# OpenDriveLab/OccNet

Hardware: AMD Instinct MI355X
Metric: nuScenes samples/sec (6-cam 900x1600 -> 200x200x16 voxels) (higher is better)
Workload: dtype f32 hot path (GEMM operands bf16x3-split, SCA value rows q16 block floating point) + bf16 backbone; 1 GPU; bevformer_base_occ forward: 6x(3x928x1600) images -> ResNet-50+FPN -> 4 BEVFormer layers (TSA+SCA+FFN) -> lifter + 2xConv3d decoder -> 200x200x16 voxels x (17 logits + 2 flow); history_frames=0, mode=infer, scope=e2e, input=resident-f32, samples_per_gpu=1, global_batch=1, parallelism=dp1, step_graph=False, linear_precision=bf16x3, backbone_dtype=bf16

## Files before the change

include/occnet_amd.h:

```cpp
#ifndef OCCNET_AMD_H_
#define OCCNET_AMD_H_

#include <stdint.h>

#ifdef __cplusplus
extern "C" {
#endif

#define OCC_OK 0
#define OCC_E_INVALID (-1)
#define OCC_E_LAUNCH (-2)
#define OCC_E_UNSUPPORTED (-3)

int occ_abi_version(void);
const char* occ_last_error(void);
int occ_selftest_fdiv_f32(const float* a, const float* d, float* q, int64_t n, void* stream);


int occ_ms_deform_attn_forward_f32(const float* value, const int64_t* spatial_shapes,
                                   const int64_t* level_start_index, const float* sampling_loc,
                                   const float* attn_weight, float* out, int B, int S, int M, int D,
                                   int L, int Lq, int P, int im2col_step, void* stream);

int occ_ms_deform_attn_backward_f32(const float* value, const int64_t* spatial_shapes,
// ... 200 lines not shown
                                    float* scale_out, void* stream);

int occ_value_proj_bf16_planes(int n_segments, const void* const* a, const int64_t* lda, const int64_t* rows,
                               const int64_t* rows_per_group, const int64_t* out_row0,
                               const float* const* group_bias, int bias_groups, const void* weight_packed, void* out,
                               int out_f16, int64_t ldo, int K, int n_planes, int plane_cols, int64_t plane_stride,
                               int64_t out_group_rows, const float* out_scale, void* stream);

int occ_stem_conv7x7_pool_f32_bf16(const float* x, const void* weight_frag, const float* bias, void* out,
                                   int batch, int H, int W, void* stream);
int occ_stem_conv7x7_pool_u8_bf16(const uint8_t* x, const void* weight_frag, const float* bias, void* out,
                                  int batch, int Hs, int Ws, int H, int W, const float* mean,
                                  const float* std, int to_rgb, void* stream);

int occ_bias_relu_maxpool_nhwc_bf16(const void* y, const float* bias, void* out, int batch, int H, int W, int C,
                                    void* stream);

int occ_conv1x1_nhwc_bf16(const void* x, const void* weight, const float* bias, const void* residual,
                          void* out, int batch, int Hin, int Win, int Cin, int Cout, int stride, int relu,
                          int residual_upsample2, void* stream);

int occ_conv1x1_nhwc_bf16_variant(const void* x, const void* weight, const float* bias, const void* residual,
                                  void* out, int batch, int Hin, int Win, int Cin, int Cout, int stride, int relu,
                                  int residual_upsample2, int variant, void* stream);

int64_t occ_conv1x1_wgrad_workspace_bytes(int N, int H, int W, int Cin, int Cout, int stride, int splits);
int occ_conv1x1_wgrad_nhwc_bf16(const void* g, const void* x, void* dw, int dw_bf16, void* workspace, int N, int H, int W,
                                int Cin, int Cout, int stride, int splits, void* stream);

int64_t occ_conv3x3_wgrad_workspace_bytes(int N, int H, int W, int Cin, int Cout, int stride, int splits);
int occ_conv3x3_wgrad_nhwc_bf16(const void* g, const void* x, void* dw, int dw_bf16, void* workspace, int N, int H, int W,
                                int Cin, int Cout, int stride, int splits, void* stream);

int occ_conv3x3_pack_weight_bf16(const float* weight, void* packed, int Cout, int Cin, void* stream);
int occ_conv3x3_nhwc_bf16(const void* x, const void* weight_packed, const float* bias, void* out, int batch,
                          int H, int W, int Cin, int Cout, int stride, int relu, void* stream);
int occ_conv3x3_nhwc_bf16_amax(const void* x, const void* weight_packed, const float* bias, void* out, int batch,
                               int H, int W, int Cin, int Cout, int stride, int relu, uint32_t* amax8, void* stream);
int occ_conv3x3_nhwc_bf16_variant(const void* x, const void* weight_packed, const float* bias, void* out, int batch,
                                  int H, int W, int Cin, int Cout, int stride, int relu, uint32_t* amax8, int variant,
                                  void* stream);

int occ_conv3x3_conv1x1_nhwc_bf16(const void* x, const void* w3x3_packed, const float* b2, const void* w1x1_frag,
                                  const float* b3, const void* residual, void* out, int batch, int H, int W, int Cmid,
                                  int Cout, int stride, int variant, void* stream);
int occ_conv3x3_conv1x1_pick(int batch, int H, int W, int Cmid, int Cout, int stride);

int occ_mfma_pack_b_frag_bf16(const float* weight, void* packed, int N, int K, void* stream);

int occ_bottleneck64_nhwc_bf16(const void* x, const void* w1_frag, const float* b1, const void* w2_frag,
                               const float* b2, const void* w3_frag, const float* b3, void* out, int batch,
                               int H, int W, int Cin, int downsample, void* stream);

int64_t occ_ray_metrics_state_words(int free_id);
int64_t occ_ray_metrics_workspace_bytes(int B, int X, int Y, int Z);
int occ_ray_metrics_accumulate(const void* sem_pred, int sem_pred_dtype, const float* flow_pred,
                               const void* sem_gt, int sem_gt_dtype, const float* flow_gt,
                               const float* origins, const int32_t* origin_counts, const float* rays,
                               float off_x, float off_y, float off_z, float voxel_size, int free_id,
                               int64_t* state, float* rows_pred, float* rows_gt, void* workspace,
                               int64_t workspace_bytes, int B, int Tmax, int X, int Y, int Z, int R,
                               void* stream);

int64_t occ_heads_loss_workspace_bytes(int64_t n_rows, int num_classes, int max_blocks);
int occ_heads_loss_fwd_f32(const float* feat, const float* w1_occ, const float* b1_occ, const float* w2_occ,
                           const float* b2_occ, const float* w1_flow, const float* b1_flow, const float* w2_flow,
                           const float* b2_flow, const void* labels, int labels_dtype, const float* flow_gt,
                           const uint8_t* mask, const float* class_weight, int64_t ignore_index, int reduction_mean,
                           float* losses, void* workspace, int64_t workspace_bytes, int64_t n_rows, int C, int hidden,
                           int num_classes, int max_blocks, void* stream);
int occ_heads_loss_bwd_f32(const float* feat, const float* w1_occ, const float* b1_occ, const float* w2_occ,
                           const float* b2_occ, const float* w1_flow, const float* b1_flow, const float* w2_flow,
                           const float* b2_flow, const void* labels, int labels_dtype, const float* flow_gt,
                           const uint8_t* mask, const float* class_weight, int64_t ignore_index, int reduction_mean,
                           const float* grad_losses, const float* occ_denom, float* dfeat, float* dw1_occ,
                           float* db1_occ, float* dw2_occ, float* db2_occ, float* dw1_flow, float* db1_flow,
                           float* dw2_flow, float* db2_flow, void* workspace, int64_t workspace_bytes, int64_t n_rows,
                           int C, int hidden, int num_classes, int max_blocks, void* stream);

#ifdef __cplusplus
}
#endif
#endif
```

occnet_amd/csrc/bottleneck64_nhwc_bf16.hip:

```cpp
#include "common.h"

namespace occ {

constexpr int kBnTH = 8, kBnTW = 16, kBnHH = 10, kBnHW = 18, kBnNP = kBnHH * kBnHW;
constexpr int kBnXS = 80;
constexpr int kBnXA = 192 * kBnXS;
constexpr int kBnMS = 144;
constexpr int kBnH1ROW = kBnHW * kBnMS;
constexpr int kBnH1 = kBnHH * kBnH1ROW;
constexpr int kBnC2 = 128 * kBnMS;
constexpr int kBnOLD = 256 + 4;

__global__ void mfma_pack_b_frag_kernel(const float* __restrict__ w, unsigned short* __restrict__ packed,
                                        int N, int K) {
  const long n_el = (long)N * K;
  const long idx = (long)blockIdx.x * blockDim.x + threadIdx.x;
  if (idx >= n_el) return;
  const int j = (int)(idx & 7), lane = (int)((idx >> 3) & 63);
  const long rest = idx >> 9;
  const int nts = N / 32;
  const int nt = (int)(rest % nts), ks = (int)(rest / nts);
  const int n = nt * 32 + (lane & 31), k = ks * 16 + (lane >> 5) * 8 + j;
  packed[idx] = bf16_rne(w[(long)n * K + k]);
}
// ... 215 lines not shown
      DST[rr] = *reinterpret_cast<const uint2*>(xs + (((long)img * H + cy) * W + cx) * CIN + c);  \
    }                                                                                             \
  }
  OCC_BN_ISSUE_RES(rn, 0)
#pragma unroll
  for (int rt = 0; rt < 4; ++rt) {
    __syncthreads();
#pragma unroll
    for (int t = 0; t < 2; ++t)
#pragma unroll
      for (int r = 0; r < 16; ++r)
        sO[((r & 3) + 8 * (r >> 2) + 4 * kb) * kBnOLD + (wave * 2 + t) * 32 + vi] = acc3[rt][t][r];
#pragma unroll
    for (int rr = 0; rr < 8; ++rr) rv[rr] = rn[rr];
    if (rt + 1 < 4) OCC_BN_ISSUE_RES(rn, rt + 1)
    __syncthreads();
#pragma unroll
    for (int rr = 0; rr < 8; ++rr) {
      const int row = wave * 8 + rr;
      const int oy = y0 + 2 * rt + (row >> 4), ox = x0 + (row & 15);
      if (oy < H && ox < W) {
        float4 v = *reinterpret_cast<const float4*>(sO + row * kBnOLD + c);
        v.x += bv.x + bf16_to_f32((unsigned short)(rv[rr].x & 0xffffu));
        v.y += bv.y + bf16_to_f32((unsigned short)(rv[rr].x >> 16));
        v.z += bv.z + bf16_to_f32((unsigned short)(rv[rr].y & 0xffffu));
        v.w += bv.w + bf16_to_f32((unsigned short)(rv[rr].y >> 16));
        v.x = fmaxf(v.x, 0.f); v.y = fmaxf(v.y, 0.f); v.z = fmaxf(v.z, 0.f); v.w = fmaxf(v.w, 0.f);
        const uint2 o = make_uint2(pack_bf16x2_rne(v.x, v.y), pack_bf16x2_rne(v.z, v.w));
        *reinterpret_cast<uint2*>(out + (((long)img * H + oy) * W + ox) * 256 + c) = o;
      }
    }
  }
#undef OCC_BN_ISSUE_RES
}

}

extern "C" int occ_mfma_pack_b_frag_bf16(const float* weight, void* packed, int N, int K, void* stream) {
  using namespace occ;
  OCC_CHECK_ARG(weight && packed, "mfma_pack_b_frag_bf16: null pointer argument");
  OCC_CHECK_ARG(N > 0 && K > 0, "mfma_pack_b_frag_bf16: bad dimension");
  if (N % 32 || K % 16) {
    set_error("mfma_pack_b_frag_bf16: N=%d K=%d (need N %% 32 == 0, K %% 16 == 0)", N, K);
    return OCC_E_UNSUPPORTED;
  }
  const long n = (long)N * K;
  hipLaunchKernelGGL(mfma_pack_b_frag_kernel, dim3((unsigned)((n + 255) / 256)), dim3(256), 0,
                     reinterpret_cast<hipStream_t>(stream), weight, reinterpret_cast<unsigned short*>(packed),
                     N, K);
  OCC_CHECK_LAUNCH("mfma_pack_b_frag_bf16");
  return OCC_OK;
}

extern "C" int occ_bottleneck64_nhwc_bf16(const void* x, const void* w1_frag, const float* b1,
                                          const void* w2_frag, const float* b2, const void* w3_frag,
                                          const float* b3, void* out, int batch, int H, int W, int Cin,
                                          int downsample, void* stream) {
  using namespace occ;
  OCC_CHECK_ARG(x && w1_frag && b1 && w2_frag && b2 && w3_frag && b3 && out,
                "bottleneck64_nhwc_bf16: null pointer argument");
  OCC_CHECK_ARG(batch > 0 && H > 0 && W > 0, "bottleneck64_nhwc_bf16: bad dimension");
  if (!((Cin == 256 && !downsample) || (Cin == 64 && downsample))) {
    set_error("bottleneck64_nhwc_bf16: no kernel for Cin=%d downsample=%d (256/identity or 64/projection)", Cin,
              downsample);
    return OCC_E_UNSUPPORTED;
  }
  const int tiles_x = (W + kBnTW - 1) / kBnTW, tiles_y = (H + kBnTH - 1) / kBnTH;
  hipStream_t st = reinterpret_cast<hipStream_t>(stream);
  const unsigned gx = (unsigned)((long)batch * tiles_x * tiles_y);
#define OCC_BN_LAUNCH(CINN, DSS)                                                                     \
  hipLaunchKernelGGL((bottleneck64_nhwc_bf16_kernel<CINN, DSS>), dim3(gx), dim3(256), 0, st,            \
                     reinterpret_cast<const uint4*>(x), reinterpret_cast<const uint4*>(w1_frag), b1,    \
                     reinterpret_cast<const uint4*>(w2_frag), b2, reinterpret_cast<const uint4*>(w3_frag), \
                     b3, reinterpret_cast<unsigned short*>(out), H, W, tiles_x, tiles_y)
  if (downsample) OCC_BN_LAUNCH(64, true); else OCC_BN_LAUNCH(256, false);
#undef OCC_BN_LAUNCH
  OCC_CHECK_LAUNCH("bottleneck64_nhwc_bf16");
  return OCC_OK;
}
```

occnet_amd/ext.py:

```python
import ctypes
import os

import torch

from . import _lib, cache_epoch
from ._lib import OccAmdError, OccAmdUnsupported, f32, i32, i64, ptr, stream_ptr


_TIMING = None
_TIMING_ONLY = None


def kernel_timing(enable=True):
    global _TIMING, _TIMING_ONLY
    _TIMING = {} if enable else None
    _TIMING_ONLY = None
    return _TIMING


def kernel_timing_only(names):
    global _TIMING_ONLY
    _TIMING_ONLY = None if names is None else set(names)


# ... 1895 lines not shown
        rc = lib.occ_conv1x1_wgrad_nhwc_bf16(ptr(g), ptr(x), ptr(dw), i32(1 if out_dtype == torch.bfloat16 else 0), ptr(ws),
                                             i32(N), i32(H), i32(W), i32(Cin), i32(Cout), i32(s), i32(sp),
                                             stream_ptr(x.device))
    _note_flops('bb_conv1x1_wgrad', 2.0 * N * g.shape[2] * g.shape[3] * Cin * Cout)
    _lib.check(rc, "conv1x1_wgrad_nhwc")
    return dw


def conv1x1_dgrad_nhwc(g, w16):
    _need_cl_bf16("conv1x1_dgrad_nhwc", "g", g)
    if not (isinstance(w16, torch.Tensor) and w16.is_cuda and w16.is_floating_point() and w16.dim() in (2, 4)
            and w16.shape[0] == g.shape[1] and w16.numel() == w16.shape[0] * w16.shape[1] and w16.device == g.device):
        raise OccAmdUnsupported("conv1x1_dgrad_nhwc: w16 must be a (Cout, Cin, 1, 1) device weight matching g's channels")
    O, I = w16.shape[0], w16.shape[1]
    with torch.cuda.device(g.device), _timed('bb_conv1x1_dgrad'):
        frag = conv1x1_pack_weight(w16.reshape(O, I).t())
        gx = conv1x1_nhwc(g, frag, torch.zeros(I, dtype=torch.float32, device=g.device), _timing=None)
    _note_flops('bb_conv1x1_dgrad', 2.0 * g.shape[0] * g.shape[2] * g.shape[3] * I * O)
    return gx


def mfma_pack_b_frag(weight2d):
    _need_cuda_f32("weight", weight2d)
    if weight2d.dim() != 2:
        raise OccAmdError("mfma_pack_b_frag: expected a (N, K) matrix")
    weight2d = weight2d.contiguous()
    n, k = weight2d.shape
    packed = torch.empty(n * k, dtype=torch.int16, device=weight2d.device)
    with torch.cuda.device(weight2d.device):
        rc = _lib.lib().occ_mfma_pack_b_frag_bf16(ptr(weight2d), ptr(packed), i32(n), i32(k),
                                                  stream_ptr(weight2d.device))
    _lib.check(rc, "mfma_pack_b_frag")
    return packed


def bottleneck64_pack(w1, b1, w2, b2, w3, b3, wds=None, bds=None):
    w1 = w1.float().reshape(w1.shape[0], -1)
    w3 = w3.float().reshape(w3.shape[0], -1)
    if tuple(w2.shape) != (64, 64, 3, 3) or w1.shape[0] != 64 or tuple(w3.shape) != (256, 64):
        raise OccAmdUnsupported("bottleneck64_pack: only 64 mid / 256 output channels")
    ds = wds is not None
    cin = w1.shape[1]
    if (ds and cin != 64) or (not ds and cin != 256):
        raise OccAmdUnsupported("bottleneck64_pack: Cin must be 256 (identity) or 64 (projection)")
    w2m = w2.float().permute(0, 2, 3, 1).reshape(64, 9 * 64)
    b3 = b3.float()
    if ds:
        w3 = torch.cat([w3, wds.float().reshape(256, 64)], dim=1)
        b3 = b3 + bds.float()
    return dict(w1=mfma_pack_b_frag(w1), b1=b1.float().contiguous(), w2=mfma_pack_b_frag(w2m),
                b2=b2.float().contiguous(), w3=mfma_pack_b_frag(w3), b3=b3.contiguous(), cin=cin, ds=ds)


def bottleneck64_nhwc(x, pack):
    _need_cl_bf16("bottleneck64_nhwc", "x", x)
    N, Cin, H, W = x.shape
    if Cin != pack['cin']:
        raise OccAmdError("bottleneck64_nhwc: x has %d channels, the pack was built for %d" % (Cin, pack['cin']))
    out = torch.empty((N, 256, H, W), dtype=torch.bfloat16, device=x.device, memory_format=torch.channels_last)
    with torch.cuda.device(x.device), _timed('bb_bottleneck64'):
        rc = _lib.lib().occ_bottleneck64_nhwc_bf16(ptr(x), ptr(pack['w1']), ptr(pack['b1']), ptr(pack['w2']),
                                                   ptr(pack['b2']), ptr(pack['w3']), ptr(pack['b3']), ptr(out),
                                                   i32(N), i32(H), i32(W), i32(Cin), i32(1 if pack['ds'] else 0),
                                                   stream_ptr(x.device))
    _note_flops('bb_bottleneck64', 2.0 * N * H * W * (Cin * 64 + 9 * 64 * 64 + 64 * 256 + (Cin * 256 if pack['ds'] else 0)))
    _lib.check(rc, "bottleneck64_nhwc")
    return out


def conv3x3_pack_weight(weight):
    _need_cuda_f32("weight", weight)
    if weight.dim() != 4 or tuple(weight.shape[2:]) != (3, 3):
        raise OccAmdError("conv3x3_pack_weight: expected a (Cout, Cin, 3, 3) weight")
    cout, cin = weight.shape[:2]
    packed = torch.empty(weight.numel(), dtype=torch.int16, device=weight.device)
    with torch.cuda.device(weight.device):
        rc = _lib.lib().occ_conv3x3_pack_weight_bf16(ptr(weight), ptr(packed), i32(cout), i32(cin),
                                                     stream_ptr(weight.device))
    _lib.check(rc, "conv3x3_pack_weight")
    return packed


def conv3x3_nhwc(x, w_packed, bias, cout, relu=False, stride=1, amax=None, variant=None):
    return _conv3x3_nhwc(x, w_packed, bias, cout, relu, stride, amax, variant, 'bb_conv3x3')


def _conv3x3_nhwc(x, w_packed, bias, cout, relu, stride, amax, variant, timing):
    _need_cl_bf16("conv3x3_nhwc", "x", x)
    _need_cuda_f32("bias", bias)
    N, Cin, H, W = x.shape
    if w_packed.numel() != cout * Cin * 9 or bias.numel() != cout:
        raise OccAmdError("conv3x3_nhwc: inconsistent shapes")
    st = int(stride)
    if st not in (1, 2):
        raise OccAmdUnsupported("conv3x3_nhwc: stride must be 1 or 2")
    if amax is not None and not (amax.is_cuda and amax.dtype == torch.int32 and amax.numel() == 8 and amax.is_contiguous()):
        raise OccAmdError("conv3x3_nhwc: amax must be 8 contiguous int32 device words")
    out = torch.empty((N, cout, (H - 1) // st + 1, (W - 1) // st + 1), dtype=torch.bfloat16, device=x.device,
                      memory_format=torch.channels_last)
    with torch.cuda.device(x.device), _timed(timing):
        rc = _lib.lib().occ_conv3x3_nhwc_bf16_variant(ptr(x), ptr(w_packed), ptr(bias), ptr(out), i32(N), i32(H),
                                                      i32(W), i32(Cin), i32(cout), i32(st), i32(1 if relu else 0),
                                                      ptr(amax), i32(0 if variant is None else int(variant)),
                                                      stream_ptr(x.device))
    _note_flops(timing, 2.0 * N * out.shape[2] * out.shape[3] * 9 * Cin * cout)
    _lib.check(rc, "conv3x3_nhwc")
    return out


def conv3x3_wgrad_nhwc(g, x, stride=1, out_dtype=torch.float32, splits=None):
    _need_cl_bf16("conv3x3_wgrad_nhwc", "g", g)
    _need_cl_bf16("conv3x3_wgrad_nhwc", "x", x)
    if out_dtype not in (torch.float32, torch.bfloat16):
        raise OccAmdUnsupported("conv3x3_wgrad_nhwc: out_dtype must be float32 or bfloat16")
    N, Cin, H, W = x.shape
    s = int(stride)
    Cout = g.shape[1]
# ... 74 lines not shown
```

occnet_amd/plugin/backbone_plan.py:

```python
import os

import torch
import torch.nn as nn
import torch.nn.functional as F
from torch.nn.utils.fusion import fuse_conv_bn_weights

from .. import ext
from .._lib import OccAmdUnsupported

_CL = torch.channels_last


def own_conv_kind(weight_shape, stride, padding, dilation=(1, 1), groups=1):
    cout, cin, kh, kw = weight_shape
    stride, padding = tuple(stride), tuple(padding)
    if tuple(dilation) != (1, 1) or groups != 1 or cin % 32:
        return None
    if (kh, kw) == (1, 1) and padding == (0, 0) and stride[0] == stride[1] and cout % 32 == 0:
        return '1x1'
    if (kh, kw) == (3, 3) and padding == (1, 1) and stride in ((1, 1), (2, 2)) and cout % 128 == 0:
        return '3x3'
    return None


# ... 112 lines not shown
            y = y + b.to(y.dtype).view(1, -1, 1, 1)
        else:
            y = F.conv2d(x, w, b.to(w.dtype), c.stride, c.padding, c.dilation, c.groups)
        if add is not None:
            y = y.add_(add)
        return y.relu_() if (relu or add is not None) else y

    @torch.no_grad()
    def forward(self, x):
        if not self.use_graph or not x.is_cuda:
            return self._forward_eager(x)
        key = (tuple(x.shape), x.dtype, str(x.device))
        st = self._graphs.setdefault(key, dict(calls=0))
        st['calls'] += 1
        if st['calls'] <= 2:
            return self._forward_eager(x)
        if 'graph' not in st:
            st['in'] = x.clone()
            torch.cuda.synchronize(x.device)
            g = torch.cuda.CUDAGraph()
            with torch.cuda.graph(g):
                st['out'] = self._forward_eager(st['in'])
            st['graph'] = g
        st['in'].copy_(x)
        st['graph'].replay()
        return st['out']

    def forward_u8(self, x_u8, mean, std, to_rgb=False, size_divisor=32):
        if not self._stem_fused:
            raise OccAmdUnsupported("forward_u8 needs the fused stem kernel (bf16 plan, 7x7/s2 stem + 3x3/s2 pool)")
        x, hw = ext.stem_conv7x7_pool_u8(x_u8, self.stem_frag, self.stem.bias, mean, std,
                                         to_rgb=to_rgb, size_divisor=size_divisor)
        return self._forward_stages(x), hw

    def _forward_eager(self, x):
        stem = self.stem
        if self._stem_fused and x.is_cuda and x.dtype == torch.float32 and x.is_contiguous():
            return self._forward_stages(ext.stem_conv7x7_pool(x, self.stem_frag, stem.bias))
        x = x.to(self.dtype).contiguous(memory_format=_CL)
        if self.hip_tail and stem.cout % 8 == 0 and x.is_cuda:
            y = F.conv2d(x, stem.weight, None, stem.stride, stem.padding, stem.dilation, stem.groups)
            if y.is_contiguous(memory_format=_CL):
                x = ext.bias_relu_maxpool_nhwc(y, stem.bias)
            else:
                x = F.max_pool2d((y + stem.bias.to(y.dtype).view(1, -1, 1, 1)).relu_(), kernel_size=3, stride=2, padding=1)
        else:
            x = F.max_pool2d(self._conv(stem, x, relu=True), kernel_size=3, stride=2, padding=1)
        return self._forward_stages(x)

    def _run_stage(self, si, x):
        for bi, (c1, c2, c3, ds) in enumerate(self.stages[si]):
            whole = self._bneck.get((si, bi))
            if whole is not None and x.is_contiguous(memory_format=_CL):
                x = ext.bottleneck64_nhwc(x, whole)
                continue
            identity = x if ds is None else self._conv(ds, x)
            y = self._conv(c1, x, relu=True)
            fused = self._conv23_fused(c2, c3, y, identity)
            x = fused if fused is not None else self._conv(c3, self._conv(c2, y, relu=True), add=identity)
        return x

    def _conv23_fused(self, c2, c3, y, identity):
        if not (c2.kind == '3x3' and c3.kind == '1x1') or os.environ.get('OCC_CONV3X3_FUSE_1X1', '1').startswith('0'):
            return None
        if not (y.is_cuda and y.dtype == torch.bfloat16 and y.is_contiguous(memory_format=_CL)
                and identity.dtype == torch.bfloat16 and identity.is_contiguous(memory_format=_CL)):
            return None
        cmid, stride = c2.cout, c2.stride[0]
        if c3.stride != (1, 1) or c3.weight.shape[1] != cmid:
            return None
        n, _, h, w = y.shape
        if not ext.conv3x3_conv1x1_pick(n, h, w, cmid, c3.cout, stride):
            return None
        return ext.conv3x3_conv1x1_nhwc(y, c2.pack, c2.bias, cmid, c3.pack, c3.bias, identity, stride=stride)

    @torch.no_grad()
    def forward_prefix(self, x):
        x = ext.stem_conv7x7_pool(x, self.stem_frag, self.stem.bias)
        for si in range(len(self.stages)):
            x = self._run_stage(si, x)
        return x

    def _forward_stages(self, x):
        feats = []
        for si in range(len(self.stages)):
            x = self._run_stage(si, x)
            if si in self.out_indices:
                feats.append(x)
        nk = self.neck
        inputs = feats
        n = len(self.laterals)
        lat = [None] * n
        nearest = nk.upsample_cfg.get('mode', 'nearest') == 'nearest' and 'scale_factor' not in nk.upsample_cfg
        for i in range(n - 1, -1, -1):
            xin = inputs[i + nk.start_level]
            li = self.laterals[i]
            up = lat[i + 1] if i + 1 < n else None
            if up is not None and nearest and li.kind == '1x1' and xin.shape[2] == 2 * up.shape[2] \
                    and xin.shape[3] == 2 * up.shape[3] and xin.is_contiguous(memory_format=_CL):
                lat[i] = ext.conv1x1_nhwc(xin, li.pack, li.bias, residual=up, relu=False, residual_upsample2=True)
                continue
            lat[i] = self._conv(li, xin)
            if up is not None:
                lat[i] = lat[i] + F.interpolate(up, size=lat[i].shape[2:], **nk.upsample_cfg)
        extra = nk.num_outs > n and bool(nk.add_extra_convs)
        srcs = list(lat)
        if extra and nk.add_extra_convs == 'on_input':
# ... 27 lines not shown
```

tools_dev/bottleneck_probe.py:

```python
import os, sys
sys.path.insert(0, os.path.join(os.path.dirname(os.path.abspath(__file__)), ".."))
import torch
from occnet_amd import ext

def run(cin, ds, iters=20):
    g = torch.Generator().manual_seed(0)
    N, H, W = 6, 232, 400
    x = torch.randn(N, cin, H, W, generator=g).cuda().to(torch.bfloat16).contiguous(memory_format=torch.channels_last)
    mk = lambda *s: torch.randn(*s, generator=g).cuda() * 0.05
    pack = ext.bottleneck64_pack(mk(64, cin, 1, 1), mk(64), mk(64, 64, 3, 3), mk(64), mk(256, 64, 1, 1), mk(256),
                                 mk(256, cin, 1, 1) if ds else None, mk(256) if ds else None)
    for _ in range(3):
        ext.bottleneck64_nhwc(x, pack)
    a, b = torch.cuda.Event(enable_timing=True), torch.cuda.Event(enable_timing=True)
    torch.cuda.synchronize(); a.record()
    for _ in range(iters):
        ext.bottleneck64_nhwc(x, pack)
    b.record(); torch.cuda.synchronize()
    us = a.elapsed_time(b) * 1e3 / iters
    mb = N * H * W * (cin + 256) * 2 / 1e6
    print(f"bottleneck64 cin={cin} ds={ds}: {us:.1f} us  ({mb:.0f} MB min traffic -> {mb / us:.2f} TB/s)")

if __name__ == '__main__':
    run(256, False); run(64, True)
```

Baseline: 195.3 samples/s.

## Add second fused bottleneck64 kernel with software-pipelined loads and tile-order remapping

Adds a new fused ResNet bottleneck kernel and makes it the default (can be turned off via env var). It prefetches x halo chunks and weights several stages ahead in registers, double-buffers the x tiles in LDS, and captures the identity residual in registers during the first GEMM. It also offers an optional block-to-tile remapping for L2 locality (order 0 is the default, so no remap). The aims are to hide global-load latency and to improve cache reuse, at the cost of more registers and a risk of lower occupancy.

```diff
diff --git a/include/occnet_amd.h b/include/occnet_amd.h
--- a/include/occnet_amd.h
+++ b/include/occnet_amd.h
@@ -276,6 +276,11 @@
                                const float* b2, const void* w3_frag, const float* b3, void* out, int batch,
                                int H, int W, int Cin, int downsample, void* stream);
 
+int occ_bottleneck64_nhwc_bf16_variant(const void* x, const void* w1_frag, const float* b1, const void* w2_frag,
+                                       const float* b2, const void* w3_frag, const float* b3, void* out, int batch,
+                                       int H, int W, int Cin, int downsample, int variant, void* stream);
+int occ_bottleneck64_tile_of_block(int block, int n_blocks, int tiles_x, int tiles_y, int order);
+
 int64_t occ_ray_metrics_state_words(int free_id);
 int64_t occ_ray_metrics_workspace_bytes(int B, int X, int Y, int Z);
 int occ_ray_metrics_accumulate(const void* sem_pred, int sem_pred_dtype, const float* flow_pred,
diff --git a/occnet_amd/csrc/bottleneck64_nhwc_bf16.hip b/occnet_amd/csrc/bottleneck64_nhwc_bf16.hip
--- a/occnet_amd/csrc/bottleneck64_nhwc_bf16.hip
+++ b/occnet_amd/csrc/bottleneck64_nhwc_bf16.hip
@@ -291,10 +291,16 @@
   return OCC_OK;
 }
 
-extern "C" int occ_bottleneck64_nhwc_bf16(const void* x, const void* w1_frag, const float* b1,
-                                          const void* w2_frag, const float* b2, const void* w3_frag,
-                                          const float* b3, void* out, int batch, int H, int W, int Cin,
-                                          int downsample, void* stream) {
+namespace occ {
+void bottleneck64_v2_launch(const void* x, const void* w1_frag, const float* b1, const void* w2_frag, const float* b2,
+                            const void* w3_frag, const float* b3, void* out, int batch, int H, int W, int downsample,
+                            int order, hipStream_t st);
+constexpr int kBnOrderDefault = 0;
+}
+
+static int bottleneck64_nhwc_bf16_launch(const void* x, const void* w1_frag, const float* b1, const void* w2_frag,
+                                         const float* b2, const void* w3_frag, const float* b3, void* out, int batch,
+                                         int H, int W, int Cin, int downsample, int variant, void* stream) {
   using namespace occ;
   OCC_CHECK_ARG(x && w1_frag && b1 && w2_frag && b2 && w3_frag && b3 && out,
                 "bottleneck64_nhwc_bf16: null pointer argument");
@@ -304,8 +310,25 @@
               downsample);
     return OCC_E_UNSUPPORTED;
   }
+  if (variant < 0 || variant > 5) {
+    set_error("bottleneck64_nhwc_bf16: no variant %d (1 = first kernel; 2 = second kernel; 3, 4, 5 = second kernel with "
+              "tile order 0, 1, 2)", variant);
+    return OCC_E_UNSUPPORTED;
+  }
+  static const bool v2_on = env_default_on("OCC_BOTTLENECK64_V2");
+  static const int order_default = [] {
+    const char* e = getenv("OCC_BOTTLENECK64_ORDER");
+    return e && e[0] >= '0' && e[0] <= '2' && !e[1] ? e[0] - '0' : kBnOrderDefault;
+  }();
+  hipStream_t st = reinterpret_cast<hipStream_t>(stream);
+  if (variant == 0) variant = v2_on ? 2 : 1;
+  if (variant != 1) {
+    bottleneck64_v2_launch(x, w1_frag, b1, w2_frag, b2, w3_frag, b3, out, batch, H, W, downsample,
+                           variant == 2 ? order_default : variant - 3, st);
+    OCC_CHECK_LAUNCH("bottleneck64_nhwc_bf16");
+    return OCC_OK;
+  }
   const int tiles_x = (W + kBnTW - 1) / kBnTW, tiles_y = (H + kBnTH - 1) / kBnTH;
-  hipStream_t st = reinterpret_cast<hipStream_t>(stream);
   const unsigned gx = (unsigned)((long)batch * tiles_x * tiles_y);
 #define OCC_BN_LAUNCH(CINN, DSS)                                                                     \
   hipLaunchKernelGGL((bottleneck64_nhwc_bf16_kernel<CINN, DSS>), dim3(gx), dim3(256), 0, st,            \
@@ -317,3 +340,19 @@
   OCC_CHECK_LAUNCH("bottleneck64_nhwc_bf16");
   return OCC_OK;
 }
+
+extern "C" int occ_bottleneck64_nhwc_bf16(const void* x, const void* w1_frag, const float* b1,
+                                          const void* w2_frag, const float* b2, const void* w3_frag,
+                                          const float* b3, void* out, int batch, int H, int W, int Cin,
+                                          int downsample, void* stream) {
+  return bottleneck64_nhwc_bf16_launch(x, w1_frag, b1, w2_frag, b2, w3_frag, b3, out, batch, H, W, Cin, downsample, 0,
+                                       stream);
+}
+
+extern "C" int occ_bottleneck64_nhwc_bf16_variant(const void* x, const void* w1_frag, const float* b1,
+                                                  const void* w2_frag, const float* b2, const void* w3_frag,
+                                                  const float* b3, void* out, int batch, int H, int W, int Cin,
+                                                  int downsample, int variant, void* stream) {
+  return bottleneck64_nhwc_bf16_launch(x, w1_frag, b1, w2_frag, b2, w3_frag, b3, out, batch, H, W, Cin, downsample,
+                                       variant, stream);
+}
diff --git a/occnet_amd/csrc/bottleneck64_v2_nhwc_bf16.hip b/occnet_amd/csrc/bottleneck64_v2_nhwc_bf16.hip
--- /dev/null
+++ b/occnet_amd/csrc/bottleneck64_v2_nhwc_bf16.hip
@@ -0,0 +1,292 @@
+#include "common.h"
+
+namespace occ {
+
+constexpr int kB2TH = 8, kB2TW = 16, kB2HH = 10, kB2HW = 18, kB2NP = kB2HH * kB2HW;
+constexpr int kB2XS = 80;
+constexpr int kB2XA = 192 * kB2XS;
+constexpr int kB2MS = 144;
+constexpr int kB2H1ROW = kB2HW * kB2MS;
+constexpr int kB2H1 = kB2HH * kB2H1ROW;
+constexpr int kB2C2 = 128 * kB2MS;
+constexpr int kB2OS = 32 * kB2MS;
+constexpr int kB2Band = 4;
+
+__host__ __device__ inline int bn64_tile_of_block(int block, int n_blocks, int tiles_x, int tiles_y, int order) {
+  if (order == 0) return block;
+  const int q = n_blocks >> 3, r = n_blocks & 7, x = block & 7, j = block >> 3;
+  const int p = x * q + (x < r ? x : r) + j;
+  if (order == 1) return p;
+  const int per_img = tiles_x * tiles_y, img = p / per_img, pi = p - img * per_img;
+  const int r0 = pi / (kB2Band * tiles_x) * kB2Band;
+  const int h = tiles_y - r0 < kB2Band ? tiles_y - r0 : kB2Band;
+  const int i = pi - r0 * tiles_x;
+  return img * per_img + (r0 + i % h) * tiles_x + i / h;
+}
+
+template <int CIN, bool DS>
+__global__ __launch_bounds__(256, 2) void bottleneck64_v2_nhwc_bf16_kernel(
+    const uint4* __restrict__ x, const uint4* __restrict__ w1p, const float* __restrict__ b1,
+    const uint4* __restrict__ w2p, const float* __restrict__ b2, const uint4* __restrict__ w3p,
+    const float* __restrict__ b3, unsigned short* __restrict__ out, int H, int W, int tiles_x, int tiles_y, int order) {
+  static_assert(CIN % 32 == 0 && (DS ? CIN == 64 : CIN == 256), "identity: 4 waves x 2 chunks; projection: both chunks in LDS");
+  constexpr int NCH = CIN / 32, CQ = CIN / 8;
+  constexpr int STAGE_BYTES = 2 * kB2XA + kB2H1 + kB2C2;
+  __shared__ __attribute__((aligned(16))) char lds[STAGE_BYTES];
+  static_assert(4 * kB2OS <= kB2H1, "the waves' epilogue scratch aliases the c1 halo");
+  char* const sH1 = lds + 2 * kB2XA;
+  char* const sC2 = sH1 + kB2H1;
+  const int tid = threadIdx.x, lane = tid & 63, wave = tid >> 6;
+  const int vi = lane & 31, kb = lane >> 5;
+  const int tile = bn64_tile_of_block((int)blockIdx.x, (int)gridDim.x, tiles_x, tiles_y, order);
+  int bid = tile;
+  const int tx_i = bid % tiles_x; bid /= tiles_x;
+  const int ty_i = bid % tiles_y;
+  const int img = bid / tiles_y;
+  const int y0 = ty_i * kB2TH, x0 = tx_i * kB2TW;
+
+  long hofs0, hofs1, hofs2;
+  int hdst0, hdst1, hdst2;
+  bool hin0, hin1, hin2, hlive0, hlive1, hlive2;
+#define OCC_B2_ROLE(K, OFS, DST, IN, LIVE)                                                        \
+  {                                                                                               \
+    const int idx = tid + 256 * (K);                                                              \
+    LIVE = idx < kB2NP * 4;                                                                       \
+    const int p = LIVE ? idx >> 2 : 0, piece = idx & 3;                                           \
+    const int hy = p / kB2HW, hx = p % kB2HW;                                                     \
+    const int iy = y0 - 1 + hy, ix = x0 - 1 + hx;                                                 \
+    IN = LIVE && iy >= 0 && iy < H && ix >= 0 && ix < W;                                          \
+    const int cy = min(max(iy, 0), H - 1), cx = min(max(ix, 0), W - 1);                           \
+    OFS = (((long)img * H + cy) * W + cx) * CQ + piece;                                           \
+    DST = p * kB2XS + piece * 16;                                                                 \
+  }
+  OCC_B2_ROLE(0, hofs0, hdst0, hin0, hlive0)
+  OCC_B2_ROLE(1, hofs1, hdst1, hin1, hlive1)
+  OCC_B2_ROLE(2, hofs2, hdst2, hin2, hlive2)
+#undef OCC_B2_ROLE
+  const unsigned hm0 = hin0 ? 0xffffffffu : 0u, hm1 = hin1 ? 0xffffffffu : 0u, hm2 = hin2 ? 0xffffffffu : 0u;
+  uint4 vh0_0, vh1_0, vh2_0, vh0_1, vh1_1, vh2_1, vh0_2, vh1_2, vh2_2, vh0_3, vh1_3, vh2_3;
+#define OCC_B2_ISSUE_X(S, CH)                                                                     \
+  {                                                                                               \
+    const long cq = (long)(CH) * 4;                                                               \
+    vh0_##S = x[hofs0 + cq]; vh1_##S = x[hofs1 + cq]; vh2_##S = x[hofs2 + cq];                    \
+  }
+  const int rot = DS ? 0 : (int)(((unsigned)tile * 5u) % (unsigned)NCH);
+#define OCC_B2_CH(CI) (((CI) + rot) % NCH)
+
+  const int ntA = wave & 1, mtA0 = 3 * (wave >> 1);
+  const int ntB = wave & 1, mtB0 = 2 * (wave >> 1);
+  float4 bA[4], bB[4];
+  f32x16 acc1[3];
+#pragma unroll
+  for (int j = 0; j < 3; ++j)
+#pragma unroll
+    for (int r = 0; r < 16; ++r) acc1[j][r] = 0.f;
+  uint2 idn[2][4][4];
+  const int wave_u = __builtin_amdgcn_readfirstlane(wave);
+  const int cbase = (((vi >> 4) + 1) * kB2HW + (vi & 15) + 1) * kB2XS + 8 * kb;
+#define OCC_B2_CAPTURE(T, SX)                                                                     \
+  _Pragma("unroll") for (int rt = 0; rt < 4; ++rt)                                                \
+    _Pragma("unroll") for (int q = 0; q < 4; ++q)                                                 \
+      idn[T][rt][q] = *reinterpret_cast<const uint2*>((SX) + cbase + rt * (2 * kB2HW * kB2XS) + 16 * q);
+  constexpr int WD = 3;
+  uint4 wa[WD][2];
+#define OCC_B2_ISSUE_W1(SLOT, CH)                                                                 \
+  {                                                                                               \
+    wa[SLOT][0] = w1p[(((long)(CH) * 2 + 0) * 2 + ntA) * 64 + lane];                              \
+    wa[SLOT][1] = w1p[(((long)(CH) * 2 + 1) * 2 + ntA) * 64 + lane];                              \
+  }
+  OCC_B2_ISSUE_W1(0, OCC_B2_CH(0))
+  OCC_B2_ISSUE_X(0, OCC_B2_CH(0))
+  OCC_B2_ISSUE_W1(1, OCC_B2_CH(NCH > 1 ? 1 : 0))
+  OCC_B2_ISSUE_X(1, OCC_B2_CH(NCH > 1 ? 1 : 0))
+  if (NCH > 2) {
+    OCC_B2_ISSUE_W1(2, OCC_B2_CH(NCH > 2 ? 2 : 0))
+    OCC_B2_ISSUE_X(2, OCC_B2_CH(NCH > 2 ? 2 : 0))
+    OCC_B2_ISSUE_X(3, OCC_B2_CH(NCH > 3 ? 3 : 0))
+  }
+#define OCC_B2_STEP_A(S, CI)                                                                      \
+  {                                                                                               \
+    char* sX = lds + ((CI) & 1) * kB2XA;                                                          \
+    if (hlive0) *reinterpret_cast<uint4*>(sX + hdst0) = make_uint4(vh0_##S.x & hm0, vh0_##S.y & hm0, vh0_##S.z & hm0, vh0_##S.w & hm0); \
+    if (hlive1) *reinterpret_cast<uint4*>(sX + hdst1) = make_uint4(vh1_##S.x & hm1, vh1_##S.y & hm1, vh1_##S.z & hm1, vh1_##S.w & hm1); \
+    if (hlive2) *reinterpret_cast<uint4*>(sX + hdst2) = make_uint4(vh2_##S.x & hm2, vh2_##S.y & hm2, vh2_##S.z & hm2, vh2_##S.w & hm2); \
+    const bf16x8 wf0 = __builtin_bit_cast(bf16x8, wa[(CI) % WD][0]), wf1 = __builtin_bit_cast(bf16x8, wa[(CI) % WD][1]); \
+    __syncthreads();                                                                              \
+    if ((CI) + WD < NCH) OCC_B2_ISSUE_W1((CI) % WD, OCC_B2_CH((CI) + WD < NCH ? (CI) + WD : NCH - 1)) \
+    if ((CI) + 4 < NCH) OCC_B2_ISSUE_X(S, OCC_B2_CH((CI) + 4 < NCH ? (CI) + 4 : NCH - 1))         \
+    if ((CI) == NCH - 2) {                                                                        \
+      _Pragma("unroll") for (int g = 0; g < 4; ++g) {                                             \
+        bA[g] = *reinterpret_cast<const float4*>(b1 + ntA * 32 + 8 * g + 4 * kb);                 \
+        bB[g] = *reinterpret_cast<const float4*>(b2 + ntB * 32 + 8 * g + 4 * kb);                 \
+      }                                                                                           \
+    }                                                                                             \
+    _Pragma("unroll") for (int j = 0; j < 3; ++j) {                                               \
+      const bf16x8 af0 = *reinterpret_cast<const bf16x8*>(sX + ((mtA0 + j) * 32 + vi) * kB2XS + kb * 16);      \
+      const bf16x8 af1 = *reinterpret_cast<const bf16x8*>(sX + ((mtA0 + j) * 32 + vi) * kB2XS + 32 + kb * 16); \
+      acc1[j] = __builtin_amdgcn_mfma_f32_32x32x16_bf16(wf0, af0, acc1[j], 0, 0, 0);              \
+      acc1[j] = __builtin_amdgcn_mfma_f32_32x32x16_bf16(wf1, af1, acc1[j], 0, 0, 0);              \
+    }                                                                                             \
+    if (!DS) {                                                                                    \
+      const int ch = OCC_B2_CH(CI);                                                               \
+      if (ch == 2 * wave_u) { OCC_B2_CAPTURE(0, sX) }                                             \
+      else if (ch == 2 * wave_u + 1) { OCC_B2_CAPTURE(1, sX) }                                    \
+    }                                                                                             \
+  }
+#pragma unroll
+  for (int ci = 0; ci < NCH; ci += 4) {
+    OCC_B2_STEP_A(0, ci)
+    if (ci + 1 < NCH) OCC_B2_STEP_A(1, ci + 1)
+    if (ci + 2 < NCH) OCC_B2_STEP_A(2, ci + 2)
+    if (ci + 3 < NCH) OCC_B2_STEP_A(3, ci + 3)
+  }
+#undef OCC_B2_STEP_A
+#undef OCC_B2_ISSUE_W1
+#undef OCC_B2_ISSUE_X
+#undef OCC_B2_CAPTURE
+#undef OCC_B2_CH
+
+  constexpr int PFB = 12;
+  uint4 wr[PFB];
+#pragma unroll
+  for (int s = 0; s < PFB; ++s) wr[s] = w2p[((long)s * 2 + ntB) * 64 + lane];
+
+#pragma unroll
+  for (int j = 0; j < 3; ++j) {
+    const int p = (mtA0 + j) * 32 + vi;
+    const int hy = p / kB2HW, hx = p - hy * kB2HW;
+    const int iy = y0 - 1 + hy, ix = x0 - 1 + hx;
+    const float m = (iy >= 0 && iy < H && ix >= 0 && ix < W) ? 1.f : 0.f;
+    if (p < kB2NP) {
+      char* dst = sH1 + p * kB2MS + (ntA * 32 + 4 * kb) * 2;
+#pragma unroll
+      for (int g = 0; g < 4; ++g) {
+        const float v0 = fmaxf(acc1[j][4 * g + 0] + bA[g].x, 0.f) * m, v1 = fmaxf(acc1[j][4 * g + 1] + bA[g].y, 0.f) * m;
+        const float v2 = fmaxf(acc1[j][4 * g + 2] + bA[g].z, 0.f) * m, v3 = fmaxf(acc1[j][4 * g + 3] + bA[g].w, 0.f) * m;
+        *reinterpret_cast<uint2*>(dst + 16 * g) = make_uint2(pack_bf16x2_rne(v0, v1), pack_bf16x2_rne(v2, v3));
+      }
+    }
+  }
+  __syncthreads();
+
+  f32x16 acc2[2];
+#pragma unroll
+  for (int j = 0; j < 2; ++j)
+#pragma unroll
+    for (int r = 0; r < 16; ++r) acc2[j][r] = 0.f;
+  const int ab0 = (2 * mtB0 + (vi >> 4)) * kB2H1ROW + (vi & 15) * kB2MS + kb * 16;
+  const int ab1 = ab0 + 2 * kB2H1ROW;
+  {
+    bf16x8 a0 = *reinterpret_cast<const bf16x8*>(sH1 + ab0), a1 = *reinterpret_cast<const bf16x8*>(sH1 + ab1);
+#pragma unroll
+    for (int s = 0; s < 36; ++s) {
+      const bf16x8 wf = __builtin_bit_cast(bf16x8, wr[s % PFB]);
+      if (s + PFB < 36) wr[s % PFB] = w2p[((long)(s + PFB) * 2 + ntB) * 64 + lane];
+      bf16x8 a0n = a0, a1n = a1;
+      if (s + 1 < 36) {
+        const int tap = (s + 1) >> 2, ks = (s + 1) & 3;
+        const int toff = (tap / 3) * kB2H1ROW + (tap % 3) * kB2MS + ks * 32;
+        a0n = *reinterpret_cast<const bf16x8*>(sH1 + ab0 + toff);
+        a1n = *reinterpret_cast<const bf16x8*>(sH1 + ab1 + toff);
+      }
+      acc2[0] = __builtin_amdgcn_mfma_f32_32x32x16_bf16(wf, a0, acc2[0], 0, 0, 0);
+      acc2[1] = __builtin_amdgcn_mfma_f32_32x32x16_bf16(wf, a1, acc2[1], 0, 0, 0);
+      __builtin_amdgcn_sched_barrier(0);
+      a0 = a0n; a1 = a1n;
+    }
+  }
+  constexpr int KS3 = DS ? 8 : 4;
+  uint4 w3f[KS3][2];
+#pragma unroll
+  for (int ks = 0; ks < KS3; ++ks)
+#pragma unroll
+    for (int t = 0; t < 2; ++t) w3f[ks][t] = w3p[((long)ks * 8 + 2 * wave + t) * 64 + lane];
+  float4 bC[2][4];
+#pragma unroll
+  for (int t = 0; t < 2; ++t)
+#pragma unroll
+    for (int q = 0; q < 4; ++q) bC[t][q] = *reinterpret_cast<const float4*>(b3 + 64 * wave + 32 * t + 8 * q + 4 * kb);
+#pragma unroll
+  for (int j = 0; j < 2; ++j) {
+    char* dst = sC2 + ((mtB0 + j) * 32 + vi) * kB2MS + (ntB * 32 + 4 * kb) * 2;
+#pragma unroll
+    for (int g = 0; g < 4; ++g) {
+      const float v0 = fmaxf(acc2[j][4 * g + 0] + bB[g].x, 0.f), v1 = fmaxf(acc2[j][4 * g + 1] + bB[g].y, 0.f);
+      const float v2 = fmaxf(acc2[j][4 * g + 2] + bB[g].z, 0.f), v3 = fmaxf(acc2[j][4 * g + 3] + bB[g].w, 0.f);
+      *reinterpret_cast<uint2*>(dst + 16 * g) = make_uint2(pack_bf16x2_rne(v0, v1), pack_bf16x2_rne(v2, v3));
+    }
+  }
+  __syncthreads();
+
+  char* const scr = sH1 + wave * kB2OS;
+  const int orow = lane >> 3, opiece = lane & 7;
+#pragma unroll
+  for (int rt = 0; rt < 4; ++rt) {
+    f32x16 acc3[2];
+#pragma unroll
+    for (int t = 0; t < 2; ++t)
+#pragma unroll
+      for (int r = 0; r < 16; ++r) acc3[t][r] = 0.f;
+#pragma unroll
+    for (int ks = 0; ks < KS3; ++ks) {
+      bf16x8 af;
+      if (ks < 4) {
+        af = *reinterpret_cast<const bf16x8*>(sC2 + (rt * 32 + vi) * kB2MS + ks * 32 + kb * 16);
+      } else {
+        const int p = (2 * rt + (vi >> 4) + 1) * kB2HW + (vi & 15) + 1;
+        af = *reinterpret_cast<const bf16x8*>(lds + ((ks - 4) >> 1) * kB2XA + p * kB2XS + ((ks - 4) & 1) * 32 + kb * 16);
+      }
+      acc3[0] = __builtin_amdgcn_mfma_f32_32x32x16_bf16(__builtin_bit_cast(bf16x8, w3f[ks][0]), af, acc3[0], 0, 0, 0);
+      acc3[1] = __builtin_amdgcn_mfma_f32_32x32x16_bf16(__builtin_bit_cast(bf16x8, w3f[ks][1]), af, acc3[1], 0, 0, 0);
+    }
+#pragma unroll
+    for (int t = 0; t < 2; ++t)
+#pragma unroll
+      for (int q = 0; q < 4; ++q) {
+        const uint2 id = DS ? make_uint2(0u, 0u) : idn[t][rt][q];
+        float v0 = acc3[t][4 * q + 0], v1 = acc3[t][4 * q + 1], v2 = acc3[t][4 * q + 2], v3 = acc3[t][4 * q + 3];
+        v0 += bC[t][q].x + bf16_lo_to_f32(id.x);
+        v1 += bC[t][q].y + bf16_hi_to_f32(id.x);
+        v2 += bC[t][q].z + bf16_lo_to_f32(id.y);
+        v3 += bC[t][q].w + bf16_hi_to_f32(id.y);
+        v0 = fmaxf(v0, 0.f); v1 = fmaxf(v1, 0.f); v2 = fmaxf(v2, 0.f); v3 = fmaxf(v3, 0.f);
+        *reinterpret_cast<uint2*>(scr + vi * kB2MS + t * 64 + q * 16 + kb * 8) =
+            make_uint2(pack_bf16x2_rne(v0, v1), pack_bf16x2_rne(v2, v3));
+      }
+    wave_lds_sync();
+#pragma unroll
+    for (int j = 0; j < 4; ++j) {
+      const int row = 8 * j + orow;
+      const int oy = y0 + 2 * rt + (row >> 4), ox = x0 + (row & 15);
+      const uint4 v = *reinterpret_cast<const uint4*>(scr + row * kB2MS + opiece * 16);
+      if (oy < H && ox < W)
+        *reinterpret_cast<uint4*>(out + (((long)img * H + oy) * W + ox) * 256 + 64 * wave + opiece * 8) = v;
+    }
+    wave_lds_sync();
+  }
+}
+
+void bottleneck64_v2_launch(const void* x, const void* w1_frag, const float* b1, const void* w2_frag, const float* b2,
+                            const void* w3_frag, const float* b3, void* out, int batch, int H, int W, int downsample,
+                            int order, hipStream_t st) {
+  const int tiles_x = (W + kB2TW - 1) / kB2TW, tiles_y = (H + kB2TH - 1) / kB2TH;
+  const unsigned gx = (unsigned)((long)batch * tiles_x * tiles_y);
+#define OCC_B2_LAUNCH(CINN, DSS)                                                                     \
+  hipLaunchKernelGGL((bottleneck64_v2_nhwc_bf16_kernel<CINN, DSS>), dim3(gx), dim3(256), 0, st,         \
+                     reinterpret_cast<const uint4*>(x), reinterpret_cast<const uint4*>(w1_frag), b1,    \
+                     reinterpret_cast<const uint4*>(w2_frag), b2, reinterpret_cast<const uint4*>(w3_frag), \
+                     b3, reinterpret_cast<unsigned short*>(out), H, W, tiles_x, tiles_y, order)
+  if (downsample) OCC_B2_LAUNCH(64, true); else OCC_B2_LAUNCH(256, false);
+#undef OCC_B2_LAUNCH
+}
+
+}
+
+extern "C" int occ_bottleneck64_tile_of_block(int block, int n_blocks, int tiles_x, int tiles_y, int order) {
+  using namespace occ;
+  OCC_CHECK_ARG(tiles_x > 0 && tiles_y > 0 && n_blocks > 0 && n_blocks % (tiles_x * tiles_y) == 0,
+                "bottleneck64_tile_of_block: n_blocks must be a positive multiple of tiles_x * tiles_y");
+  OCC_CHECK_ARG(block >= 0 && block < n_blocks, "bottleneck64_tile_of_block: block outside 0 .. n_blocks - 1");
+  OCC_CHECK_ARG(order >= 0 && order <= 2, "bottleneck64_tile_of_block: order must be 0, 1 or 2");
+  return bn64_tile_of_block(block, n_blocks, tiles_x, tiles_y, order);
+}
diff --git a/occnet_amd/ext.py b/occnet_amd/ext.py
--- a/occnet_amd/ext.py
+++ b/occnet_amd/ext.py
@@ -1971,17 +1971,22 @@
                 b2=b2.float().contiguous(), w3=mfma_pack_b_frag(w3), b3=b3.contiguous(), cin=cin, ds=ds)
 
 
-def bottleneck64_nhwc(x, pack):
+def bottleneck64_nhwc(x, pack, variant=0, out=None):
     _need_cl_bf16("bottleneck64_nhwc", "x", x)
     N, Cin, H, W = x.shape
     if Cin != pack['cin']:
         raise OccAmdError("bottleneck64_nhwc: x has %d channels, the pack was built for %d" % (Cin, pack['cin']))
-    out = torch.empty((N, 256, H, W), dtype=torch.bfloat16, device=x.device, memory_format=torch.channels_last)
+    if out is None:
+        out = torch.empty((N, 256, H, W), dtype=torch.bfloat16, device=x.device, memory_format=torch.channels_last)
+    else:
+        _need_cl_bf16("bottleneck64_nhwc", "out", out)
+        if tuple(out.shape) != (N, 256, H, W) or out.device != x.device or out.data_ptr() == x.data_ptr():
+            raise OccAmdError("bottleneck64_nhwc: out must be a (N, 256, H, W) tensor on x's device, not x itself")
     with torch.cuda.device(x.device), _timed('bb_bottleneck64'):
-        rc = _lib.lib().occ_bottleneck64_nhwc_bf16(ptr(x), ptr(pack['w1']), ptr(pack['b1']), ptr(pack['w2']),
-                                                   ptr(pack['b2']), ptr(pack['w3']), ptr(pack['b3']), ptr(out),
-                                                   i32(N), i32(H), i32(W), i32(Cin), i32(1 if pack['ds'] else 0),
-                                                   stream_ptr(x.device))
+        rc = _lib.lib().occ_bottleneck64_nhwc_bf16_variant(ptr(x), ptr(pack['w1']), ptr(pack['b1']), ptr(pack['w2']),
+                                                           ptr(pack['b2']), ptr(pack['w3']), ptr(pack['b3']), ptr(out),
+                                                           i32(N), i32(H), i32(W), i32(Cin), i32(1 if pack['ds'] else 0),
+                                                           i32(int(variant)), stream_ptr(x.device))
     _note_flops('bb_bottleneck64', 2.0 * N * H * W * (Cin * 64 + 9 * 64 * 64 + 64 * 256 + (Cin * 256 if pack['ds'] else 0)))
     _lib.check(rc, "bottleneck64_nhwc")
     return out
diff --git a/occnet_amd/plugin/backbone_plan.py b/occnet_amd/plugin/backbone_plan.py
--- a/occnet_amd/plugin/backbone_plan.py
+++ b/occnet_amd/plugin/backbone_plan.py
@@ -188,7 +188,8 @@
         for bi, (c1, c2, c3, ds) in enumerate(self.stages[si]):
             whole = self._bneck.get((si, bi))
             if whole is not None and x.is_contiguous(memory_format=_CL):
-                x = ext.bottleneck64_nhwc(x, whole)
+                first = os.environ.get('OCC_BOTTLENECK64_V2', '1').startswith('0')
+                x = ext.bottleneck64_nhwc(x, whole, variant=1 if first else 0)
                 continue
             identity = x if ds is None else self._conv(ds, x)
             y = self._conv(c1, x, relu=True)
diff --git a/tools_dev/bottleneck_pmc.py b/tools_dev/bottleneck_pmc.py
--- /dev/null
+++ b/tools_dev/bottleneck_pmc.py
@@ -0,0 +1,69 @@
+#!/usr/bin/env python
+import argparse
+import collections
+import csv
+import glob
+import os
+import subprocess
+import sys
+import tempfile
+
+SETS = ["FETCH_SIZE", "WRITE_SIZE", "TCC_HIT_sum TCC_MISS_sum", "SQ_WAVE_CYCLES SQ_WAIT_INST_ANY SQ_BUSY_CYCLES",
+        "SQ_VALU_MFMA_BUSY_CYCLES TA_TA_BUSY_sum"]
+ROOT = os.path.dirname(os.path.dirname(os.path.abspath(__file__)))
+
+
+def main():
+    ap = argparse.ArgumentParser()
+    ap.add_argument('--variants', default='1,3,4,5')
+    ap.add_argument('--out', default=None, help='also write the table to this file')
+    a = ap.parse_args()
+    variants = [int(v) for v in a.variants.split(',')]
+    iters = 2
+    order = [1] + variants + [v for v in variants for _ in range(3 + iters)]
+    acc = collections.defaultdict(lambda: [0, 0.0])
+    for i, cset in enumerate(SETS):
+        d = tempfile.mkdtemp(prefix='bnpmc_')
+        cmd = ['rocprofv3', '--pmc'] + cset.split() + ['--kernel-trace', '--output-format', 'csv',
+               '--kernel-include-regex', 'bottleneck64', '-d', d, '-o', 'p', '--', sys.executable,
+               os.path.join(ROOT, 'tools_dev', 'bottleneck_probe.py'), '--variants', a.variants, '--iters', str(iters),
+               '--rounds', '1']
+        res = subprocess.run(cmd, capture_output=True, text=True, timeout=240, cwd=d)
+        if res.returncode != 0:
+            sys.stderr.write(res.stdout[-2000:] + res.stderr[-2000:])
+            raise SystemExit(f"rocprofv3 failed on counter set {cset!r} (exit {res.returncode})")
+        paths = glob.glob(os.path.join(d, '**', '*counter_collection.csv'), recursive=True)
+        if not paths:
+            raise SystemExit(f"no counter_collection.csv for {cset!r}")
+        rows = [r for p in paths for r in csv.DictReader(open(p))]
+        for cin, tag in ((256, '<256, false>'), (64, '<64, true>')):
+            ids = sorted({int(r['Dispatch_Id']) for r in rows if tag in r['Kernel_Name']})
+            if len(ids) != len(order):
+                raise SystemExit(f"{len(ids)} launches of {tag}, expected {len(order)}")
+            which = dict(zip(ids, order))
+            for r in rows:
+                if tag in r['Kernel_Name']:
+                    v = which[int(r['Dispatch_Id'])]
+                    assert ('_v2_' in r['Kernel_Name']) == (v != 1), (r['Kernel_Name'], v)
+                    k = acc[(cin, v, r['Counter_Name'])]
+                    k[0] += 1
+                    k[1] += float(r['Counter_Value'])
+    lines = ["# rocprofv3 --pmc (one counter set per run, kernel trace only) over tools_dev/bottleneck_probe.py, 6 x 232 x 400;",
+             "# mean per launch.  variant 1 = first kernel, 3 / 4 / 5 = second kernel with tile order 0 / 1 / 2.",
+             "# FETCH_SIZE / WRITE_SIZE in KB as rocprofv3 reports them (bytes read = 2 x FETCH_SIZE x 1024, as profiles/ computes it)"]
+    names = sorted({c for (_, _, c) in acc})
+    for cin in (256, 64):
+        lines.append(f"cin {cin}")
+        lines.append(f"  {'counter':28s}" + ''.join(f"{'variant ' + str(v):>16s}" for v in variants))
+        for c in names:
+            lines.append(f"  {c:28s}" + ''.join(f"{acc[(cin, v, c)][1] / max(acc[(cin, v, c)][0], 1):16.5g}" for v in variants))
+    text = '\n'.join(lines) + '\n'
+    if a.out:
+        os.makedirs(os.path.dirname(os.path.abspath(a.out)), exist_ok=True)
+        with open(a.out, 'w') as f:
+            f.write(text)
+    print(text)
+
+
+if __name__ == '__main__':
+    main()
diff --git a/tools_dev/bottleneck_probe.py b/tools_dev/bottleneck_probe.py
--- a/tools_dev/bottleneck_probe.py
+++ b/tools_dev/bottleneck_probe.py
@@ -1,25 +1,53 @@
-import os, sys
+import argparse
+import os
+import sys
 sys.path.insert(0, os.path.join(os.path.dirname(os.path.abspath(__file__)), ".."))
 import torch
 from occnet_amd import ext
 
-def run(cin, ds, iters=20):
+
+def setup(cin, ds):
     g = torch.Generator().manual_seed(0)
     N, H, W = 6, 232, 400
     x = torch.randn(N, cin, H, W, generator=g).cuda().to(torch.bfloat16).contiguous(memory_format=torch.channels_last)
     mk = lambda *s: torch.randn(*s, generator=g).cuda() * 0.05
     pack = ext.bottleneck64_pack(mk(64, cin, 1, 1), mk(64), mk(64, 64, 3, 3), mk(64), mk(256, 64, 1, 1), mk(256),
                                  mk(256, cin, 1, 1) if ds else None, mk(256) if ds else None)
-    for _ in range(3):
-        ext.bottleneck64_nhwc(x, pack)
-    a, b = torch.cuda.Event(enable_timing=True), torch.cuda.Event(enable_timing=True)
-    torch.cuda.synchronize(); a.record()
-    for _ in range(iters):
-        ext.bottleneck64_nhwc(x, pack)
-    b.record(); torch.cuda.synchronize()
-    us = a.elapsed_time(b) * 1e3 / iters
+    return x, pack
+
+
+def run(cin, ds, variants, iters, rounds):
+    x, pack = setup(cin, ds)
+    N, _, H, W = x.shape
     mb = N * H * W * (cin + 256) * 2 / 1e6
-    print(f"bottleneck64 cin={cin} ds={ds}: {us:.1f} us  ({mb:.0f} MB min traffic -> {mb / us:.2f} TB/s)")
+    ref = ext.bottleneck64_nhwc(x, pack, variant=1)
+    out = torch.empty_like(ref)
+    for v in variants:
+        same = torch.equal(ext.bottleneck64_nhwc(x, pack, variant=v), ref)
+        print(f"bottleneck64 cin={cin} ds={ds} variant {v}: bits equal to variant 1: {same}")
+    for r in range(rounds):
+        for v in variants:
+            for _ in range(3):
+                ext.bottleneck64_nhwc(x, pack, variant=v, out=out)
+            a, b = torch.cuda.Event(enable_timing=True), torch.cuda.Event(enable_timing=True)
+            torch.cuda.synchronize(); a.record()
+            for _ in range(iters):
+                ext.bottleneck64_nhwc(x, pack, variant=v, out=out)
+            b.record(); torch.cuda.synchronize()
+            us = a.elapsed_time(b) * 1e3 / iters
+            print(f"bottleneck64 cin={cin} ds={ds} variant {v} round {r}: {us:.1f} us  "
+                  f"({mb:.0f} MB min traffic -> {mb / us:.2f} TB/s)", flush=True)
+
 
 if __name__ == '__main__':
-    run(256, False); run(64, True)
+    ap = argparse.ArgumentParser()
+    ap.add_argument('--variants', default='1,2')
+    ap.add_argument('--iters', type=int, default=20)
+    ap.add_argument('--rounds', type=int, default=3)
+    ap.add_argument('--only', choices=['256', '64'], default=None)
+    a = ap.parse_args()
+    vs = [int(v) for v in a.variants.split(',')]
+    if a.only != '64':
+        run(256, False, vs, a.iters, a.rounds)
+    if a.only != '256':
+        run(64, True, vs, a.iters, a.rounds)
```

New measurement: 197.6 samples/s, median of 6. 1.01x the previous value.
